# quokka-astro/quokka

Measured on AMD Instinct MI355X. Metric: Mcell-updates/s on 3D Sedov unigrid, higher is better.
Workload: dtype f64; 1 GPU; 3D Sedov blast 256x256x256 unigrid (tests/blast_unigrid_256.in scaled to 256^3 cells per GPU), 128^3 boxes, PPM+HLLC RK2, gamma=1.4, CFL 0.3, reflecting octant; cells_per_gpu=16777216, boxes_per_gpu=8, parallelism=box-decomposition x1, rk2_mode=carry, fofc_stages=0, retries=0, x_sweep_in_y_march=True

## Files before the change

### quokka_amd/csrc/qk_hydro_fused.hip

```cpp
#include "qk_device.hpp"
#include <algorithm>
#include <cmath>
#include <cstdlib>
#include <type_traits>
#include <vector>

#include "qk_internal.hpp"

using namespace qk;

namespace
{

constexpr int NG = 4;

template <class P> QK_DEV void streamStore(P *p, double v) { __builtin_nontemporal_store(v, p); }
template <class P> QK_DEV auto streamLoad(P *p) -> double { return __builtin_nontemporal_load(p); }

struct SGeom {
	int64_t off;
	int glo[3];
	int n[3];
	int pitch;
	int64_t ncell;
// ... 501 lines not shown
QK_DEV auto epiTgas(Eos const &eos, EpiConst const &ec, Recip const &Rrho, double Eint) -> double
{
	if (eos.tmodel == 1) {
		return sqrt(sqrt(4.0 * Eint / eos.alpha));
	}
	const double e = divBy(Eint, Rrho);
	const double T = divBy(e * eos.mu * Eos::m_u * eos.gm1, ec.RkB);
	return divBy(T * Eos::k_B, ec.RkBu);
}
QK_DEV auto epiEint(Eos const &eos, EpiConst const &ec, double rho, double T) -> double
{
	if (eos.tmodel == 1) {
		return (eos.alpha / 4.0) * ((T * T) * (T * T));
	}
	const double p = divBy(rho * T * Eos::k_B, ec.Rmu);
	const double e = p / (eos.gm1 * rho);
	return divBy(e * rho * eos.kB_user, ec.RkB);
}

template <int NS, int CS, bool FOFC = false, int NDIM = 3>
QK_DEV void updateCellFrom(SweepArgs const &a, Eos const &eos, EpiConst const &ec, int b, int i, int j, int k, double U[NVAR + NS], const double rhs_sweeps[NVAR + NS],
			   double div_v, const double half[NVAR + NS + 1], double &sig0, double &sig1, bool haveP = false, double Pknown = 0.)
{
	WA4 Un(a.U_out[b]);
	IA4 flag(a.redoFlag[b]);
	if constexpr (FOFC) {
		if (flag(i, j, k) != 0) {
			div_v = cellCentredDivV<NDIM>(RA4(a.U_old[b]), i, j, k, a.dx3);
		}
	}
	double rhs[NVAR + NS];
#pragma unroll
	for (int n = 0; n < NVAR + NS; ++n) {
		rhs[n] = rhs_sweeps[n];
	}
	double Pgas;
	if (CS == 2) {
		Pgas = half[NVAR + NS];
	} else if (haveP) {
		Pgas = Pknown;
	} else {
		const double rho = U[RHO];
		if (eos.isothermal) {
			Pgas = rho * eos.cs_iso * eos.cs_iso;
		} else {
			const Recip Ro = recipOf(rho);
			const double vx = divBy(U[MX], Ro), vy = divBy(U[MY], Ro), vz = divBy(U[MZ], Ro);
			const double thermal_energy = U[ENE] - 0.5 * rho * (vx * vx + vy * vy + vz * vz);
			const double e = (rho == 0.0) ? 0.0 : divBy(thermal_energy, Ro);
			Pgas = eos.gm1 * rho * e;
		}
	}
	double r[NVAR];
#pragma unroll
	for (int n = 0; n < NVAR; ++n) {
		r[n] = rhs[n];
	}
	r[EINT] += -Pgas * div_v;
	if (CS == 1) {
		WA4 R1(a.rhs1[b]);
		const int64_t c1 = R1.idx(i, j, k);
		const double hdt = 0.5 * a.dt;
#pragma unroll
		for (int n = 0; n < NVAR + NS; ++n) {
			streamStore(&R1.p[c1 + R1.ns * n], U[n] + hdt * ((n < NVAR) ? r[n] : rhs[n]));
		}
		streamStore(&R1.p[c1 + R1.ns * (NVAR + NS)], Pgas);
	}
	if (CS == 2) {
		const double hdt = 0.5 * a.dt;
#pragma unroll
		for (int n = 0; n < NVAR + NS; ++n) {
			U[n] = half[n] + hdt * ((n < NVAR) ? r[n] : rhs[n]);
		}
	} else {
#pragma unroll
		for (int n = 0; n < NVAR; ++n) {
			U[n] = U[n] + a.dt * r[n];
		}
#pragma unroll
		for (int n = NVAR; n < NVAR + NS; ++n) {
			U[n] = U[n] + a.dt * rhs[n];
		}
	}
	const int bad = (U[RHO] > 0.) ? 0 : 1;
	if constexpr (!FOFC) {
		flag(i, j, k) = bad;
	}
	if (bad != 0) {
		atomicAdd(a.redo_count, 1ULL);
	}
	const bool fix = FOFC || (bad == 0);
	double rho_new = U[RHO];
	if (fix && U[RHO] < a.densityFloor) {
#pragma unroll
		for (int n = NVAR; n < NVAR + NS; ++n) {
			U[n] = (a.densityFloor == 0.0) ? 0.0 : U[n] * (U[RHO] / a.densityFloor);
		}
		rho_new = a.densityFloor;
		U[RHO] = rho_new;
	}
	const Recip Rn = recipOf(rho_new);
	const double px = U[MX], py = U[MY], pz = U[MZ];
	const double vx = divBy(px, Rn), vy = divBy(py, Rn), vz = divBy(pz, Rn);
	if (fix) {
		if ((rho_new > 2.2250738585072014e-308) && !eos.isothermal) {
			const double Ekin = 0.5 * rho_new * (vx * vx + vy * vy + vz * vz);
			const double Etot = U[ENE];
			if (epiTgas(eos, ec, Rn, Etot - Ekin) < a.tempFloor) {
				U[ENE] = Ekin + epiEint(eos, ec, rho_new, a.tempFloor);
			}
			if (epiTgas(eos, ec, Rn, U[EINT]) < a.tempFloor) {
				U[EINT] = epiEint(eos, ec, rho_new, a.tempFloor);
			}
		}
	}
	const double Ekin2 = 0.5 * divBy(px * px + py * py + pz * pz, Rn);
	if constexpr (FOFC) {
		if (a.use_dual_energy != 0 && !(rho_new > 0.)) {
			*a.error_flag = 1;
		}
	}
	if (fix && a.use_dual_energy != 0 && (!FOFC || rho_new > 0.)) {
		const double Etot = U[ENE];
		const double Eint_aux = U[EINT];
		const double Eint_cons = Etot - Ekin2;
		if (Eint_cons > 1.0e-3 * Etot) {
			U[EINT] = Eint_cons;
		} else {
			U[EINT] = Eint_aux;
			U[ENE] = Eint_aux + Ekin2;
		}
	}
	const int64_t cn = Un.idx(i, j, k);
	if (a.prim_out) {
		const double Eint_cons = U[ENE] - 0.5 * rho_new * (vx * vx + vy * vy + vz * vz);
		const double e = (rho_new == 0.0) ? 0.0 : divBy(Eint_cons, Rn);
		streamStore(&Un.p[cn + Un.ns * PRHO], rho_new);
		streamStore(&Un.p[cn + Un.ns * PVX], vx);
		streamStore(&Un.p[cn + Un.ns * PVY], vy);
		streamStore(&Un.p[cn + Un.ns * PVZ], vz);
		streamStore(&Un.p[cn + Un.ns * PPRES], eos.gm1 * rho_new * e);
		streamStore(&Un.p[cn + Un.ns * PEINT], U[EINT]);
#pragma unroll
		for (int n = NVAR; n < NVAR + NS; ++n) {
			streamStore(&Un.p[cn + Un.ns * n], U[n]);
		}
	} else {
#pragma unroll
		for (int n = 0; n < NVAR + NS; ++n) {
			streamStore(&Un.p[cn + Un.ns * n], U[n]);
		}
	}
	if (a.max_signal != nullptr) {
		double cs;
		if (eos.isothermal) {
			cs = eos.cs_iso;
		} else {
			const double thermal_energy = U[ENE] - 0.5 * rho_new * (vx * vx + vy * vy + vz * vz);
			const double e = (rho_new == 0.0) ? 0.0 : divBy(thermal_energy, Rn);
			const double P = eos.gm1 * rho_new * e;
			cs = sqrtN(divBy(eos.gamma * P, Rn));
		}
		sig0 = smax(sig0, cs + sqrtN(divBy(2.0 * Ekin2, Rn)));
		sig1 = smax(sig1, cs + sqrtN(vx * vx + vy * vy + vz * vz));
	}
}

#ifndef QK_XB
#define QK_XB 256
#endif
constexpr int XB = QK_XB;
constexpr int XOUT = XB - 6;

template <int ORDER, int STAGE, int NS, bool CARRY, int NDIM = 3, bool FOFC = false> __global__ void __launch_bounds__(XB) k_sweep_x(SweepArgs a, Eos eos)
{
	static_assert(!(FOFC && CARRY), "the first-order flux correction pass exists for the reference's form of the RK2 average");
	constexpr int NV = NVAR + NS;
	constexpr int RHS_DIVV = S_RHS + NV;
	__shared__ double s_q[NV][XB];
	__shared__ double s_e[NV][XB];
	__shared__ double s_d[3][XB];

	const int b = blockIdx.z;
	const qk_box bx = a.boxes[b];
	const SGeom g = a.geom[b];
	const int t = threadIdx.x;
	const int k = bx.lo[2] + blockIdx.y;
	if (k > bx.hi[2]) {
		return;
	}
	const int64_t rowlen = g.n[0];
	const int64_t slablen = rowlen * (bx.hi[1] - bx.lo[1] + 1);
	const int64_t f = static_cast<int64_t>(blockIdx.x) * XOUT + t - 3;
	const bool inside = (f >= 0) && (f < slablen);
	const int jj = static_cast<int>((inside ? f : 0) / rowlen);
	const int i = g.glo[0] + static_cast<int>((inside ? f : 0) - jj * rowlen);
	const int j = bx.lo[1] + jj;
	const int64_t c = (i - g.glo[0]) + static_cast<int64_t>(g.pitch) * ((j - g.glo[1]) + static_cast<int64_t>(g.n[1]) * (k - g.glo[2]));

	const double *S = a.scratch + g.off;
	const int64_t T = a.total_cells;
	double q0[NV], Uc[NVAR];
	{
		RA4 U(a.U_in[b]);
		loadPrims<NS>(U, U.idx(i, j, k), eos, a.reconstruct_eint, a.prim_in, q0, Uc);
	}
	putColumn(s_q, t, q0);
	const double chi = S[(S_AUX + 0) * T + c];
	const double dV = S[(S_AUX + 2) * T + c];
	const double dW = S[(S_AUX + 3) * T + c];
	s_d[0][t] = dV;
	s_d[1][t] = dW;
	__syncthreads();

	double am[NV], ap[NV];
	const int tm1 = max(t - 1, 0), tp1 = min(t + 1, XB - 1);
	reconstructCell<ORDER>(chi, q0, [&](int m, int n) { return s_q[n][min(max(t + m, 0), XB - 1)]; }, am, ap);
	putColumn(s_e, t, ap);
	__syncthreads();

	double qL[NV];
	getColumn(s_e, tm1, qL);
	const double du = q0[PVX] - s_q[PVX][tm1];
	const double dvl = s_d[0][tm1], dwl = s_d[1][tm1];
	double F[NV], vf;
	faceFluxAll<0, QK_RIEMANN_HLLC, false, NS>(eos, a.reconstruct_eint, NDIM, qL, am, du, dvl, dV, dwl, dW, a.K_visc, F, vf);

	const bool validRow = inside;
	const bool isFace = validRow && (i >= bx.lo[0]) && (i <= bx.hi[0] + 1) && (t >= 3) && (t <= XB - 3);
	if (isFace) {
		const int fi[3] = {i, j, k};
		double F1[NV + 1];
		if (!CARRY && STAGE == 2) {
			loadF1<NV>(a, b, fi, F1);
		}
		bool marked = false;
		if (CARRY && a.fluxMask != nullptr) {
			const qk_carray4 md = a.fluxMask[b];
			marked = (maskByte(md, i - 1, j, k) | maskByte(md, i, j, k)) != 0;
		}
		double qLo[NV];
		if (FOFC && STAGE == 1) {
			getColumn(s_q, tm1, qLo);
		}
		settleFace<STAGE, CARRY, FOFC, 0, NS, false>(a, eos, NDIM, b, fi, true, marked, F1, qLo, q0, F, vf);
	}
	__syncthreads();
	putColumn(s_q, t, F);
	s_d[2][t] = vf;
	__syncthreads();

	const bool isCell = validRow && (i >= bx.lo[0]) && (i <= bx.hi[0]) && (t >= 3) && (t < 3 + XOUT);
	if constexpr (NDIM == 1) {
		double sig0 = 0., sig1 = 0.;
		if (isCell) {
			double rhs[NV], r1[NV + 1];
#pragma unroll
			for (int n = 0; n < NV; ++n) {
				rhs[n] = a.inv_dx * (F[n] - s_q[n][tp1]);
				r1[n] = 0.;
			}
			r1[NV] = 0.;
			const double div_v = (s_d[2][tp1] - vf) / a.dx;
			RA4 Uold(a.U_old[b]);
			const int64_t co = Uold.idx(i, j, k);
			double Uo[NV];
#pragma unroll
			for (int n = 0; n < NV; ++n) {
				Uo[n] = Uold.p[co + Uold.ns * n];
			}
			if (CARRY && STAGE == 2) {
				RA4 R1(a.rhs1[b]);
				const int64_t c1 = R1.idx(i, j, k);
#pragma unroll
				for (int n = 0; n < NV + 1; ++n) {
					r1[n] = R1.p[c1 + R1.ns * n];
				}
			}
			const EpiConst ec = epiConst(eos);
			updateCellFrom<NS, CARRY ? STAGE : 0, FOFC, 1>(a, eos, ec, b, i, j, k, Uo, rhs, div_v, r1, sig0, sig1);
		}
		if (a.max_signal != nullptr) {
			reduceSignal(a.max_signal, sig0, sig1);
		}
	} else if (isCell) {
		double *R = a.scratch + g.off + c;
#pragma unroll
		for (int n = 0; n < NV; ++n) {
			streamStore(&R[(S_RHS + n) * T], a.inv_dx * (F[n] - s_q[n][tp1]));
		}
		R[RHS_DIVV * T] = (s_d[2][tp1] - vf) / a.dx;
	}
}

#ifndef QK_MARCH_BY
#define QK_MARCH_BY 4
#endif
constexpr int MARCH_BY = QK_MARCH_BY;
constexpr int XW = 64 + 8;
#ifndef QK_XROWS
#define QK_XROWS 16
#endif
constexpr int XROWS = QK_XROWS;
static_assert(XROWS == 8 || XROWS == 16 || XROWS == 32, "the batch maps rows and sides onto the lanes of one wave");
QK_DEV void waveFence()
{
	__builtin_amdgcn_fence(__ATOMIC_SEQ_CST, "wavefront");
	__builtin_amdgcn_wave_barrier();
}
template <int NV> using EdgeRow = double[6][NV + 1];
template <int NV> QK_DEV void stageEdgeRow(double (*sx)[XW], const EdgeRow<NV> &row)
{
	const int t6 = static_cast<int>(threadIdx.x);
	if (t6 < 6) {
		const int slot = (t6 < 2) ? t6 : 64 + t6;
#pragma unroll
		for (int n = 0; n < NV + 1; ++n) {
			sx[n][slot] = row[t6][n];
		}
	}
}
template <int ORDER, int NS>
QK_DEV void fusexEdgeBatch(SweepArgs const &a, Eos const &eos, RA4 const &Uin, SGeom const &g, const int64_t (&st)[3], const double *S, int x0, int row0, int hi, int ot, EdgeRow<NVAR + NS> *edge)
{
	constexpr int NV = NVAR + NS;
	const int64_t T = a.total_cells;
	const int tx = static_cast<int>(threadIdx.x);
	const int side = (tx / XROWS) & 1;
	const int brow = tx & (XROWS - 1);
	const int mrow = min(row0 + brow, hi);
	const int f = x0 + 64 * side;
	int64_t ub = Uin.idx(f - 3, mrow, ot);
	double qb[6][NV], Uc[NVAR];
#pragma unroll
	for (int m = 0; m < 6; ++m, ++ub) {
		loadPrims<NS>(Uin, ub, eos, a.reconstruct_eint, a.prim_in, qb[m], Uc);
	}
	const int64_t cb = (f - 1 - g.glo[0]) + (mrow - g.glo[1]) * st[1] + (ot - g.glo[2]) * st[2];
	const double chiL = S[cb], chiR = S[cb + 1];
	const double DyL = S[(S_AUX + 2) * T + cb], DyR = S[(S_AUX + 2) * T + cb + 1];
	const double DzL = S[(S_AUX + 3) * T + cb], DzR = S[(S_AUX + 3) * T + cb + 1];
	double qLb[NV], qRb[NV], Fb[NV], vfb;
#pragma unroll
	for (int n = 0; n < NV; ++n) {
		double unused;
		reconstructVar<ORDER>(chiL, qb[0][n], qb[1][n], qb[2][n], qb[3][n], qb[4][n], unused, qLb[n]);
		reconstructVar<ORDER>(chiR, qb[1][n], qb[2][n], qb[3][n], qb[4][n], qb[5][n], qRb[n], unused);
	}
	faceFluxAll<0, QK_RIEMANN_HLLC, false, NS>(eos, a.reconstruct_eint, 3, qLb, qRb, qb[3][PVX] - qb[2][PVX], DyL, DyR, DzL, DzR, a.K_visc, Fb, vfb);
	double(*ed)[NV + 1] = edge[brow];
	double *ef = ed[5 - side];
#pragma unroll
	for (int n = 0; n < NV; ++n) {
		ef[n] = Fb[n];
	}
	ef[NV] = vfb;
#pragma unroll
	for (int n = 0; n < NV; ++n) {
		ed[2 * side][n] = (side != 0) ? qb[3][n] : qb[1][n];
		ed[2 * side + 1][n] = (side != 0) ? qb[4][n] : qb[2][n];
	}
}
template <int DIR, int ORDER, int STAGE, bool LAST, int NS, bool CARRY, bool TWOD = false, bool FOFC = false, bool FUSEX = false>
__global__ void __launch_bounds__(64 * MARCH_BY) k_sweep_march(SweepArgs a, Eos eos)
{
	static_assert(!FUSEX || (DIR == 1 && !LAST && !TWOD && !FOFC && CARRY), "the X sweep rides on the Y sweep of a 3-D level in the carried form");
	static_assert(!(FOFC && CARRY), "the first-order flux correction pass exists for the reference's form of the RK2 average");
	static_assert(!TWOD || (DIR == 1 && LAST), "the 2-D build has one marching sweep: y, carrying the epilogue");
	constexpr int NV = NVAR + NS;
	constexpr int RHS_DIVV = S_RHS + NV;
	static_assert(DIR == 1 || DIR == 2, "marching sweeps are the strided directions");
	const BlockId blk = xcdContiguousBlock();
	const int bix = blk.x, biy = blk.y, biz = blk.z;
	const int b = biz / a.nseg;
	const int seg = biz - b * a.nseg;
	const qk_box bx = a.boxes[b];
	const SGeom g = a.geom[b];
	constexpr int OT = (DIR == 1) ? 2 : 1;
	const int i_raw = bx.lo[0] + bix * 64 + threadIdx.x;
	const int ot_raw = bx.lo[OT] + biy * MARCH_BY + threadIdx.y;
	const bool live = (i_raw <= bx.hi[0]) && (ot_raw <= bx.hi[OT]);
	const int i = min(i_raw, bx.hi[0]);
	const int ot = min(ot_raw, bx.hi[OT]);
	double sig0 = 0., sig1 = 0.;
	const int64_t T = a.total_cells;
	const int64_t st[3] = {1, g.pitch, static_cast<int64_t>(g.pitch) * g.n[1]};
	const int64_t ms = st[DIR];
	const int seglen = (bx.hi[DIR] - bx.lo[DIR] + 1 + a.nseg - 1) / a.nseg;
	const int lo = bx.lo[DIR] + seg * seglen, hi = min(lo + seglen - 1, bx.hi[DIR]);
	const int nvalid = hi - lo + 1;
	if (nvalid <= 0) {
		return;
	}
	if constexpr (FUSEX) {
		if (bx.lo[0] + bix * 64 > bx.hi[0]) {
			return;
		}
	}
	int pos[3];
	pos[0] = i;
	pos[OT] = ot;
	pos[DIR] = lo - 3;
	int64_t c = (pos[0] - g.glo[0]) * st[0] + (pos[1] - g.glo[1]) * st[1] + (pos[2] - g.glo[2]) * st[2];
	const double *S = a.scratch + g.off;
	double *Sw = a.scratch + g.off;
	RA4 Uin(a.U_in[b]);
	RA4 Uold(a.U_old[b]);
	const EpiConst ec = epiConst(eos);
	int64_t u = Uin.idx(pos[0], pos[1], pos[2]);
	const int64_t ums = (DIR == 1) ? Uin.js : Uin.ks;

	constexpr int AV = Axes<DIR, TWOD>::v, AW = Axes<DIR, TWOD>::w;
	double q[5][NV];
	double apPrev[NV], Fprev[NV];
	double vfPrev = 0., dVprev = 0., dWprev = 0.;
	bool maskCol = false;
	int maskLo = 0, maskHi = -1;
	if (CARRY && a.fluxMask != nullptr) {
		const qk_carray4 md = a.fluxMask[b];
		maskCol = live && i >= md.begin[0] && i < md.end[0] && ot >= md.begin[OT] && ot < md.end[OT];
		maskLo = md.begin[DIR];
		maskHi = md.end[DIR] - 1;
	}
	constexpr bool RING = LAST && (STAGE == 1);
	__shared__ double s_ring[RING ? 3 : 1][RING ? NV : 1][RING ? 64 * MARCH_BY : 1];
	__shared__ double s_fx[FUSEX ? MARCH_BY : 1][FUSEX ? NV + 2 : 1][FUSEX ? XW : 1];
	__shared__ double s_edge[FUSEX ? MARCH_BY : 1][FUSEX ? XROWS : 1][6][FUSEX ? NV + 1 : 1];
	double chiPrev = 1.;
	const int lself = (FUSEX && threadIdx.x == 0) ? 69 : static_cast<int>(threadIdx.x) + 2;
	const int lnext = (FUSEX && threadIdx.x == 63) ? 68 : static_cast<int>(threadIdx.x) + 3;
	const int tid = threadIdx.y * 64 + threadIdx.x;
	const bool ring = RING && a.same_old;
	int slot = 0;
	double Uo[NV];
#pragma unroll
	for (int n = 0; n < NV; ++n) {
		apPrev[n] = 0.;
		Fprev[n] = 0.;
#pragma unroll
		for (int m = 0; m < 5; ++m) {
			q[m][n] = 0.;
		}
	}

	constexpr bool PFQ = !FUSEX && NS == 0;
	double Un[NVAR];
	if constexpr (PFQ) {
#pragma unroll
		for (int n = 0; n < NVAR; ++n) {
			Un[n] = Uin.p[u + Uin.ns * n];
		}
	}
	for (int step = 0; step < nvalid + 6; ++step, c += ms, u += ums) {
#pragma unroll
		for (int n = 0; n < NV; ++n) {
			q[0][n] = q[1][n];
			q[1][n] = q[2][n];
			q[2][n] = q[3][n];
			q[3][n] = q[4][n];
		}
		{
			double Uc[NVAR];
			if constexpr (PFQ) {
#pragma unroll
				for (int n = 0; n < NVAR; ++n) {
					Uc[n] = Un[n];
					Un[n] = Uin.p[u + ums + Uin.ns * n];
				}
				primsOf<NS>(Uin, u, eos, a.reconstruct_eint, a.prim_in, Uc, q[4]);
			} else {
				loadPrims<NS>(Uin, u, eos, a.reconstruct_eint, a.prim_in, q[4], Uc);
			}
			if constexpr (RING) {
				if (ring) {
#pragma unroll
					for (int n = 0; n < NV; ++n) {
						Uo[n] = s_ring[slot][n][tid];
						s_ring[slot][n][tid] = (n < NVAR) ? Uc[n] : q[4][n];
					}
					slot = (slot == 2) ? 0 : slot + 1;
				}
			}
		}
		if (step < 4) {
			continue;
		}
		const int64_t cc = c - 2 * ms;
		const double chi = S[(S_AUX + 0) * T + cc];
		const double dV = S[(S_AUX + 1 + AV) * T + cc];
		const double dW = S[(S_AUX + 1 + AW) * T + cc];
		int fidx[3], cidx[3];
		fidx[0] = cidx[0] = i;
		fidx[OT] = cidx[OT] = ot;
		fidx[DIR] = lo + (step - 5);
		cidx[DIR] = lo + (step - 6);
		const int64_t cu = cc - ms;
		double rhs_in[NV + 1], F1[NV + 1];
		if (step >= 6) {
			if constexpr (FUSEX) {
				double(*sx)[XW] = s_fx[threadIdx.y];
				EdgeRow<NV> *edge = s_edge[threadIdx.y];
				const int rr = (step - 6) & (XROWS - 1);
				if (rr == 0) {
					fusexEdgeBatch<ORDER, NS>(a, eos, Uin, g, st, S, bx.lo[0] + bix * 64, cidx[DIR], hi, ot, edge);
					waveFence();
					stageEdgeRow<NV>(sx, edge[0]);
				}
				const double Dy = S[(S_AUX + 2) * T + cu];
				const int l = static_cast<int>(threadIdx.x) + 2;
				putColumn(sx, l, q[1]);
				waveFence();
				double amx[NV], apx[NV];
				reconstructCell<ORDER>(chiPrev, q[1], [&](int m, int n) { return sx[n][l + m]; }, amx, apx);
				const double uLeft = sx[PVX][l - 1];
				waveFence();
				putColumn(sx, l, apx);
				sx[NV][l] = Dy;
				sx[NV + 1][l] = dVprev;
				waveFence();
				double qLx[NV], Fx[NV], vfx;
				getColumn(sx, l - 1, qLx);
				const double dvl = sx[NV][l - 1], dwl = sx[NV + 1][l - 1];
				faceFluxAll<0, QK_RIEMANN_HLLC, false, NS>(eos, a.reconstruct_eint, 3, qLx, amx, q[1][PVX] - uLeft, dvl, Dy, dwl, dVprev, a.K_visc, Fx, vfx);
				waveFence();
				putColumn(sx, l, Fx);
				sx[NV][l] = vfx;
				waveFence();
#pragma unroll
				for (int n = 0; n < NV; ++n) {
					rhs_in[n] = a.inv_dx0 * (sx[n][lself] - sx[n][lnext]);
				}
				rhs_in[NV] = (sx[NV][lnext] - sx[NV][lself]) / a.dx0;
				waveFence();
				if (rr + 1 < XROWS) {
					stageEdgeRow<NV>(sx, edge[rr + 1]);
				}
			} else {
#pragma unroll
				for (int n = 0; n < NV + 1; ++n) {
					rhs_in[n] = streamLoad(&S[(S_RHS + n) * T + cu]);
				}
			}
			if (LAST && !ring && !(CARRY && STAGE == 2)) {
				const int64_t co = Uold.idx(cidx[0], cidx[1], cidx[2]);
#pragma unroll
				for (int n = 0; n < NV; ++n) {
					Uo[n] = Uold.p[co + Uold.ns * n];
				}
			}
			if (CARRY && LAST && STAGE == 2) {
				RA4 R1(a.rhs1[b]);
				const int64_t c1 = R1.idx(cidx[0], cidx[1], cidx[2]);
#pragma unroll
				for (int n = 0; n < NV + 1; ++n) {
					F1[n] = R1.p[c1 + R1.ns * n];
				}
			}
		}
		if (!CARRY && STAGE == 2 && step >= 5) {
			loadF1<NV>(a, b, fidx, F1);
		}
		double am[NV], ap[NV];
		reconstructCell<ORDER>(chi, q[2], [&](int m, int n) { return q[2 + m][n]; }, am, ap);
		if (step >= 5) {
			const double du = q[2][PVX + DIR] - q[1][PVX + DIR];
			double F[NV], vf;
			faceFluxAll<DIR, QK_RIEMANN_HLLC, TWOD, NS>(eos, a.reconstruct_eint, TWOD ? 2 : 3, apPrev, am, du, dVprev, dV, dWprev, dW, a.K_visc, F, vf);
			bool marked = false;
			if (maskCol && fidx[DIR] >= maskLo && cidx[DIR] <= maskHi) {
				CA4 M(a.fluxMask[b]);
				const int m0 = (cidx[DIR] >= maskLo) ? M(cidx[0], cidx[1], cidx[2]) : 0;
				const int m1 = (fidx[DIR] <= maskHi) ? M(fidx[0], fidx[1], fidx[2]) : 0;
				marked = (m0 | m1) != 0;
			}
			settleFace<STAGE, CARRY, FOFC, DIR, NS, TWOD>(a, eos, TWOD ? 2 : 3, b, fidx, live, marked, F1, q[1], q[2], F, vf);
			if (step >= 6) {
				double rhs[NV];
#pragma unroll
				for (int n = 0; n < NV; ++n) {
					rhs[n] = rhs_in[n] + a.inv_dx * (Fprev[n] - F[n]);
				}
				const double div_v = rhs_in[NV] + (vf - vfPrev) / a.dx;
				if (LAST) {
					if (live) {
						updateCellFrom<NS, CARRY ? STAGE : 0, FOFC, TWOD ? 2 : 3>(a, eos, ec, b, cidx[0], cidx[1], cidx[2], Uo, rhs, div_v, F1, sig0, sig1,
													    (STAGE == 1) && a.same_old && !a.reconstruct_eint && !a.prim_in, q[1][PPRES]);
					}
				} else if (live) {
#pragma unroll
					for (int n = 0; n < NV; ++n) {
						streamStore(&Sw[(S_RHS + n) * T + cu], rhs[n]);
					}
					streamStore(&Sw[RHS_DIVV * T + cu], div_v);
				}
			}
#pragma unroll
			for (int n = 0; n < NV; ++n) {
				Fprev[n] = F[n];
			}
			vfPrev = vf;
		}
#pragma unroll
		for (int n = 0; n < NV; ++n) {
			apPrev[n] = ap[n];
		}
		dVprev = dV;
		dWprev = dW;
		chiPrev = chi;
	}
	if (LAST && a.max_signal != nullptr) {
		reduceSignal(a.max_signal, sig0, sig1);
	}
}

inline auto smallLevelCells() -> int64_t
{
	static const int64_t v = [] {
		const char *e = std::getenv("QK_SMALL_LEVEL_CELLS");
		return (e != nullptr) ? static_cast<int64_t>(std::atoll(e)) : static_cast<int64_t>(2) << 20;
	}();
	return v;
}

inline auto smallMinLen() -> int
{
	static const int v = [] {
		const char *e = std::getenv("QK_SMALL_MINLEN");
		return (e != nullptr) ? std::max(1, std::atoi(e)) : 4;
	}();
	return v;
}

auto marchSegments(const qk_level *lev, int dir, int ot) -> int
{
	if (const char *e = std::getenv("QK_MARCH_SEGMENTS")) {
		return std::max(1, std::atoi(e));
	}
	const int64_t cols = static_cast<int64_t>(lev->nboxes) * lev->maxlen[0] * lev->maxlen[ot];
	const int64_t want = (131072 + cols - 1) / std::max<int64_t>(cols, 1);
	const int minlen = (cols * lev->maxlen[dir] < smallLevelCells()) ? smallMinLen() : 16;
	const int cap = std::max(1, lev->maxlen[dir] / minlen);
	return static_cast<int>(std::min<int64_t>(std::max<int64_t>(want, 1), std::min(cap, 16)));
}

inline auto rowAlign() -> bool
{
	static const bool v = [] {
		const char *e = std::getenv("QK_ROW_ALIGN");
		return e == nullptr || std::atoi(e) == 1 || std::atoi(e) == 3;
	}();
	return v;
}

auto scratchGeom(const qk_level *lev, std::vector<SGeom> &g) -> int64_t
{
	g.resize(lev->nboxes);
	const bool al = rowAlign();
	int64_t off = 0;
	for (int b = 0; b < lev->nboxes; ++b) {
		for (int d = 0; d < 3; ++d) {
			g[b].glo[d] = lev->boxes[b].lo[d] - NG;
			g[b].n[d] = lev->boxes[b].hi[d] - lev->boxes[b].lo[d] + 1 + 2 * NG;
		}
		g[b].pitch = al ? (g[b].n[0] + 15) / 16 * 16 : g[b].n[0];
		if (al) {
			off = (off + 15) / 16 * 16 + (16 - NG);
		}
		g[b].off = off;
		g[b].ncell = static_cast<int64_t>(g[b].pitch) * g[b].n[1] * g[b].n[2];
		off += g[b].ncell;
	}
	return al ? (off + 15) / 16 * 16 : off;
}

auto buildGeom(qk_level *lev) -> int
{
	if (lev->d_sgeom != nullptr) {
		return QK_OK;
	}
	std::vector<SGeom> g;
	const int64_t total = scratchGeom(lev, g);
	void *d = nullptr;
	QK_HIP_CHECK(lev->ctx, hipMalloc(&d, sizeof(SGeom) * lev->nboxes));
	QK_HIP_CHECK(lev->ctx, hipMemcpy(d, g.data(), sizeof(SGeom) * lev->nboxes, hipMemcpyHostToDevice));
	lev->d_sgeom = d;
	lev->sgeom_total_cells = total;
	return QK_OK;
}

auto prePassSegments(const qk_level *lev, int xt, int yt) -> int
{
	if (const char *e = std::getenv("QK_PRE_SEGMENTS")) {
		return std::max(1, std::atoi(e));
	}
	const bool small = static_cast<int64_t>(lev->nboxes) * lev->maxlen[0] * lev->maxlen[1] * lev->maxlen[2] < smallLevelCells();
	const int64_t tiles = static_cast<int64_t>(xt) * yt * lev->nboxes;
	const int nplanes = lev->maxlen[2] + 2;
	if (small) {
		return static_cast<int>(std::min<int64_t>((1024 + tiles - 1) / tiles, std::max(1, nplanes / smallMinLen())));
	}
	const int base = std::max(1, std::min(8, (nplanes + 15) / 30));
	int nseg = base;
	const double slots = 512.0;
	if (static_cast<double>(tiles) * base / slots < 6.0) {
		double best = 1e300;
		for (int c = std::max(1, base - 1); c <= base + 1; ++c) {
			const double rounds = static_cast<double>(tiles) * c / slots;
			const int seglen = (nplanes + c - 1) / c;
			const double cost = (std::ceil(rounds) / rounds) * (static_cast<double>(seglen + 6) / seglen);
			if (cost < best) {
				best = cost;
				nseg = c;
			}
		}
	}
	return nseg;
}

auto sweepArgsFor(SweepArgs a, const qk_hydro_stage_args *args, int d) -> SweepArgs
{
	a.halfFlux = args->halfFlux[d];
	a.halfVel = args->halfVel[d];
	a.rk2Flux = args->fluxRk2[d];
	a.inv_dx = 1.0 / args->dx[d];
	a.dx = args->dx[d];
	return a;
}

auto fusexApplies(const qk_level *lev, SweepArgs const &a, bool carry, int nscalars) -> bool
{
	const char *e = std::getenv("QK_FUSEX");
	if (!carry || nscalars != 0 || lev->ndim != 3 || a.fluxMask != nullptr || (e != nullptr && std::atoi(e) == 0)) {
		return false;
	}
	for (int b = 0; b < lev->nboxes; ++b) {
		if ((lev->boxes[b].hi[0] - lev->boxes[b].lo[0] + 1) % 64 != 0) {
			return false;
		}
	}
	return true;
}

template <int ORDER, int STAGE, int NS, bool CARRY, bool FOFC = false> void launchSweeps(qk_level *lev, hipStream_t s, SweepArgs a, Eos eos, const qk_hydro_stage_args *args)
{
	const bool fusex = fusexApplies(lev, a, CARRY, NS);
	if (!fusex) {
		const SweepArgs ax = sweepArgsFor(a, args, 0);
		const int64_t slab = static_cast<int64_t>(lev->maxlen[0] + 2 * NG) * lev->maxlen[1];
		const dim3 grid(static_cast<unsigned>((slab + XOUT - 1) / XOUT), static_cast<unsigned>(lev->maxlen[2]), static_cast<unsigned>(lev->nboxes));
		ProfScope ps(lev->ctx, s, "k_sweep_x");
		if (lev->ndim == 3) {
			hipLaunchKernelGGL((k_sweep_x<ORDER, STAGE, NS, CARRY, 3, FOFC>), grid, dim3(XB), 0, s, ax, eos);
		} else if constexpr (!CARRY) {
			if (lev->ndim == 2) {
				hipLaunchKernelGGL((k_sweep_x<ORDER, STAGE, NS, false, 2, FOFC>), grid, dim3(XB), 0, s, ax, eos);
			} else {
				hipLaunchKernelGGL((k_sweep_x<ORDER, STAGE, NS, false, 1, FOFC>), grid, dim3(XB), 0, s, ax, eos);
			}
		}
	}
	if (lev->ndim == 1) {
		return;
	}
	{
		SweepArgs ay = sweepArgsFor(a, args, 1);
		ay.same_old = (lev->ndim == 2) && (args->U_in == args->U_old);
		ay.nseg = marchSegments(lev, 1, 2);
		ay.inv_dx0 = 1.0 / args->dx[0];
		ay.dx0 = args->dx[0];
		const dim3 grid((lev->maxlen[0] + 63) / 64, (lev->maxlen[2] + MARCH_BY - 1) / MARCH_BY, lev->nboxes * ay.nseg);
		ProfScope ps(lev->ctx, s, fusex ? "k_sweep_xy" : "k_sweep_y");
		if (lev->ndim == 2) {
			if constexpr (!CARRY) {
				hipLaunchKernelGGL((k_sweep_march<1, ORDER, STAGE, true, NS, false, true, FOFC>), grid, dim3(64, MARCH_BY), 0, s, ay, eos);
			}
			return;
		}
		if constexpr (CARRY && !FOFC && NS == 0) {
			if (fusex) {
				hipLaunchKernelGGL((k_sweep_march<1, ORDER, STAGE, false, NS, CARRY, false, FOFC, true>), grid, dim3(64, MARCH_BY), 0, s, ay, eos);
			}
		}
		if (!fusex) {
			hipLaunchKernelGGL((k_sweep_march<1, ORDER, STAGE, false, NS, CARRY, false, FOFC>), grid, dim3(64, MARCH_BY), 0, s, ay, eos);
		}
	}
	{
		SweepArgs az = sweepArgsFor(a, args, 2);
		az.same_old = (args->U_in == args->U_old);
		az.nseg = marchSegments(lev, 2, 1);
		const dim3 grid((lev->maxlen[0] + 63) / 64, (lev->maxlen[1] + MARCH_BY - 1) / MARCH_BY, lev->nboxes * az.nseg);
		ProfScope ps(lev->ctx, s, "k_sweep_z");
		hipLaunchKernelGGL((k_sweep_march<2, ORDER, STAGE, true, NS, CARRY, false, FOFC>), grid, dim3(64, MARCH_BY), 0, s, az, eos);
	}
}

template <int ORDER, int NS> void launchStage(qk_level *lev, hipStream_t s, SweepArgs const &a, Eos const &eos, const qk_hydro_stage_args *args)
{
	auto form = [&](auto stage) {
		constexpr int STAGE = decltype(stage)::value;
		if (args->fofc_pass != 0) {
			launchSweeps<ORDER, STAGE, NS, false, true>(lev, s, a, eos, args);
		} else if (args->rk2_carry_rhs != 0) {
			launchSweeps<ORDER, STAGE, NS, true>(lev, s, a, eos, args);
		} else {
			launchSweeps<ORDER, STAGE, NS, false>(lev, s, a, eos, args);
		}
	};
	if (args->stage == 1) {
		form(std::integral_constant<int, 1>{});
// ... 149 lines not shown
```

Before: 3208 Mcell-updates/s.

## Prefetch conserved state and aux fields in fused X-in-Y march, stage edge batch via LDS

Turns on the next-row conserved-variable prefetch for the fused X-in-Y sweep and adds a one-step-ahead prefetch of chi and the transverse divergence aux fields. This hides global-load latency behind the current step's work. The edge-batch routine now stages its primitives through a new shared buffer instead of a 6xNV register array, or reads them directly when inputs are already primitive. The batch call is also moved to the top of the loop. The aim is lower register pressure and load latency, at the cost of more LDS, extra registers for the prefetched values, and one extra wave fence.

```diff
diff --git a/quokka_amd/csrc/qk_hydro_fused.hip b/quokka_amd/csrc/qk_hydro_fused.hip
--- a/quokka_amd/csrc/qk_hydro_fused.hip
+++ b/quokka_amd/csrc/qk_hydro_fused.hip
@@ -827,6 +827,12 @@
 #ifndef QK_XROWS
 #define QK_XROWS 16
 #endif
+#ifndef QK_XY_PFQ
+#define QK_XY_PFQ 1
+#endif
+#ifndef QK_XY_PFAUX
+#define QK_XY_PFAUX 1
+#endif
 constexpr int XROWS = QK_XROWS;
 static_assert(XROWS == 8 || XROWS == 16 || XROWS == 32, "the batch maps rows and sides onto the lanes of one wave");
 QK_DEV void waveFence()
@@ -846,46 +852,62 @@
 		}
 	}
 }
+template <int NV> using BatchCells = double[6][NV][2 * XROWS];
 template <int ORDER, int NS>
-QK_DEV void fusexEdgeBatch(SweepArgs const &a, Eos const &eos, RA4 const &Uin, SGeom const &g, const int64_t (&st)[3], const double *S, int x0, int row0, int hi, int ot, EdgeRow<NVAR + NS> *edge)
+QK_DEV void fusexEdgeBatch(SweepArgs const &a, Eos const &eos, RA4 const &Uin, SGeom const &g, const int64_t (&st)[3], const double *S, int x0, int row0, int hi, int ot, EdgeRow<NVAR + NS> *edge,
+			   BatchCells<NVAR + NS> &bq)
 {
 	constexpr int NV = NVAR + NS;
 	const int64_t T = a.total_cells;
 	const int tx = static_cast<int>(threadIdx.x);
+	const int bl = tx & (2 * XROWS - 1);
 	const int side = (tx / XROWS) & 1;
 	const int brow = tx & (XROWS - 1);
 	const int mrow = min(row0 + brow, hi);
 	const int f = x0 + 64 * side;
-	int64_t ub = Uin.idx(f - 3, mrow, ot);
-	double qb[6][NV], Uc[NVAR];
-#pragma unroll
-	for (int m = 0; m < 6; ++m, ++ub) {
-		loadPrims<NS>(Uin, ub, eos, a.reconstruct_eint, a.prim_in, qb[m], Uc);
+	const int64_t ub = Uin.idx(f - 3, mrow, ot);
+	if (!a.prim_in) {
+#pragma unroll
+		for (int m = 0; m < 6; ++m) {
+			double qc[NV], Uc[NVAR];
+			loadPrims<NS>(Uin, ub + m, eos, a.reconstruct_eint, false, qc, Uc);
+#pragma unroll
+			for (int n = 0; n < NV; ++n) {
+				bq[m][n][bl] = qc[n];
+			}
+		}
+		waveFence();
 	}
 	const int64_t cb = (f - 1 - g.glo[0]) + (mrow - g.glo[1]) * st[1] + (ot - g.glo[2]) * st[2];
 	const double chiL = S[cb], chiR = S[cb + 1];
+	double(*ed)[NV + 1] = edge[brow];
+	double qLb[NV], qRb[NV], du = 0.;
+#pragma unroll
+	for (int n = 0; n < NV; ++n) {
+		double v[6];
+#pragma unroll
+		for (int m = 0; m < 6; ++m) {
+			v[m] = a.prim_in ? Uin.p[ub + m + Uin.ns * n] : bq[m][n][bl];
+		}
+		double unused;
+		reconstructVar<ORDER>(chiL, v[0], v[1], v[2], v[3], v[4], unused, qLb[n]);
+		reconstructVar<ORDER>(chiR, v[1], v[2], v[3], v[4], v[5], qRb[n], unused);
+		if (n == PVX) {
+			du = v[3] - v[2];
+		}
+		ed[2 * side][n] = (side != 0) ? v[3] : v[1];
+		ed[2 * side + 1][n] = (side != 0) ? v[4] : v[2];
+	}
 	const double DyL = S[(S_AUX + 2) * T + cb], DyR = S[(S_AUX + 2) * T + cb + 1];
 	const double DzL = S[(S_AUX + 3) * T + cb], DzR = S[(S_AUX + 3) * T + cb + 1];
-	double qLb[NV], qRb[NV], Fb[NV], vfb;
-#pragma unroll
-	for (int n = 0; n < NV; ++n) {
-		double unused;
-		reconstructVar<ORDER>(chiL, qb[0][n], qb[1][n], qb[2][n], qb[3][n], qb[4][n], unused, qLb[n]);
-		reconstructVar<ORDER>(chiR, qb[1][n], qb[2][n], qb[3][n], qb[4][n], qb[5][n], qRb[n], unused);
-	}
-	faceFluxAll<0, QK_RIEMANN_HLLC, false, NS>(eos, a.reconstruct_eint, 3, qLb, qRb, qb[3][PVX] - qb[2][PVX], DyL, DyR, DzL, DzR, a.K_visc, Fb, vfb);
-	double(*ed)[NV + 1] = edge[brow];
+	double Fb[NV], vfb;
+	faceFluxAll<0, QK_RIEMANN_HLLC, false, NS>(eos, a.reconstruct_eint, 3, qLb, qRb, du, DyL, DyR, DzL, DzR, a.K_visc, Fb, vfb);
 	double *ef = ed[5 - side];
 #pragma unroll
 	for (int n = 0; n < NV; ++n) {
 		ef[n] = Fb[n];
 	}
 	ef[NV] = vfb;
-#pragma unroll
-	for (int n = 0; n < NV; ++n) {
-		ed[2 * side][n] = (side != 0) ? qb[3][n] : qb[1][n];
-		ed[2 * side + 1][n] = (side != 0) ? qb[4][n] : qb[2][n];
-	}
 }
 template <int DIR, int ORDER, int STAGE, bool LAST, int NS, bool CARRY, bool TWOD = false, bool FOFC = false, bool FUSEX = false>
 __global__ void __launch_bounds__(64 * MARCH_BY) k_sweep_march(SweepArgs a, Eos eos)
@@ -952,6 +974,7 @@
 	__shared__ double s_ring[RING ? 3 : 1][RING ? NV : 1][RING ? 64 * MARCH_BY : 1];
 	__shared__ double s_fx[FUSEX ? MARCH_BY : 1][FUSEX ? NV + 2 : 1][FUSEX ? XW : 1];
 	__shared__ double s_edge[FUSEX ? MARCH_BY : 1][FUSEX ? XROWS : 1][6][FUSEX ? NV + 1 : 1];
+	__shared__ double s_bq[FUSEX ? MARCH_BY : 1][FUSEX ? 6 : 1][FUSEX ? NV : 1][FUSEX ? 2 * XROWS : 1];
 	double chiPrev = 1.;
 	const int lself = (FUSEX && threadIdx.x == 0) ? 69 : static_cast<int>(threadIdx.x) + 2;
 	const int lnext = (FUSEX && threadIdx.x == 63) ? 68 : static_cast<int>(threadIdx.x) + 3;
@@ -969,7 +992,9 @@
 		}
 	}
 
-	constexpr bool PFQ = !FUSEX && NS == 0;
+	constexpr bool PFQ = (!FUSEX || QK_XY_PFQ != 0) && NS == 0;
+	constexpr bool PFA = FUSEX && PFQ && QK_XY_PFAUX != 0;
+	double chiN = 1., dVN = 0., dWN = 0.;
 	double Un[NVAR];
 	if constexpr (PFQ) {
 #pragma unroll
@@ -978,6 +1003,13 @@
 		}
 	}
 	for (int step = 0; step < nvalid + 6; ++step, c += ms, u += ums) {
+		if constexpr (FUSEX) {
+			if (step >= 6 && ((step - 6) & (XROWS - 1)) == 0) {
+				fusexEdgeBatch<ORDER, NS>(a, eos, Uin, g, st, S, bx.lo[0] + bix * 64, lo + (step - 6), hi, ot, s_edge[threadIdx.y], s_bq[threadIdx.y]);
+				waveFence();
+				stageEdgeRow<NV>(s_fx[threadIdx.y], s_edge[threadIdx.y][0]);
+			}
+		}
 #pragma unroll
 		for (int n = 0; n < NV; ++n) {
 			q[0][n] = q[1][n];
@@ -1008,13 +1040,26 @@
 				}
 			}
 		}
+		const int64_t cc = c - 2 * ms;
+		double chi, dV, dW;
+		if constexpr (PFA) {
+			chi = chiN;
+			dV = dVN;
+			dW = dWN;
+			if (step >= 3) {
+				chiN = S[(S_AUX + 0) * T + cc + ms];
+				dVN = S[(S_AUX + 1 + AV) * T + cc + ms];
+				dWN = S[(S_AUX + 1 + AW) * T + cc + ms];
+			}
+		}
 		if (step < 4) {
 			continue;
 		}
-		const int64_t cc = c - 2 * ms;
-		const double chi = S[(S_AUX + 0) * T + cc];
-		const double dV = S[(S_AUX + 1 + AV) * T + cc];
-		const double dW = S[(S_AUX + 1 + AW) * T + cc];
+		if constexpr (!PFA) {
+			chi = S[(S_AUX + 0) * T + cc];
+			dV = S[(S_AUX + 1 + AV) * T + cc];
+			dW = S[(S_AUX + 1 + AW) * T + cc];
+		}
 		int fidx[3], cidx[3];
 		fidx[0] = cidx[0] = i;
 		fidx[OT] = cidx[OT] = ot;
@@ -1027,11 +1072,6 @@
 				double(*sx)[XW] = s_fx[threadIdx.y];
 				EdgeRow<NV> *edge = s_edge[threadIdx.y];
 				const int rr = (step - 6) & (XROWS - 1);
-				if (rr == 0) {
-					fusexEdgeBatch<ORDER, NS>(a, eos, Uin, g, st, S, bx.lo[0] + bix * 64, cidx[DIR], hi, ot, edge);
-					waveFence();
-					stageEdgeRow<NV>(sx, edge[0]);
-				}
 				const double Dy = S[(S_AUX + 2) * T + cu];
 				const int l = static_cast<int>(threadIdx.x) + 2;
 				putColumn(sx, l, q[1]);
```

Result: no change. 3235 Mcell-updates/s, median of 6 (+0.8%).
